# wwood/smafa

Hardware: AMD Instinct MI355X
Metric: query seqs/sec (DB residues/sec in `residues_per_s`) vs roofline, 10M x 60aa DB, d<=5 (higher is better)
Workload: dtype u32

## Files before the change

### smafa_amd/csrc/kernels.hip.h

```cpp
#pragma once

#include <type_traits>
#include <hip/hip_runtime.h>
#include <stdint.h>

#include "../../include/smafa_amd.h"
#include "scan_plan.h"

namespace smafa {

constexpr int kStageRows = 256;
__host__ __device__ constexpr int scan_min_waves(int ps, int w, int t) {
    const int regs = t * ps * w * 4 + 40;
    return regs <= 64 ? 8 : regs <= 80 ? 6 : regs <= 96 ? 5 : regs <= 128 ? 4 : regs <= 168 ? 3 : 2;
}
#ifndef SMAFA_CASCADE
#define SMAFA_CASCADE 1
#endif
#ifndef SMAFA_WIDE_AND_PAIR
#define SMAFA_WIDE_AND_PAIR 1
#endif
#ifndef SMAFA_SIGN_COMPARE
#define SMAFA_SIGN_COMPARE 1
#endif
// ... 863 lines not shown
#pragma unroll
        for (int t = 0; t < T; t++) {
            const bool live = (uint32_t)t < n_live;
            uint4 f1;
            if constexpr (kF1Home == 2) f1 = f1_reg[t];
            else f1 = planes[(size_t)(live ? tile0 + t : a.tile_begin) * (PS * W * 64) + (FP * W + 1) * 64 + lane];
            if constexpr (kF1Home == 1) f1_home[t * 64 + lane] = f1;
            const uint32_t w0[4] = {f0[t].x, f0[t].y, f0[t].z, f0[t].w};
            const uint32_t w1[4] = {f1.x, f1.y, f1.z, f1.w};
#pragma unroll
            for (int k = 0; k < 4; k++) {
                const uint32_t ky = key_y(w0[k]), kx = key_x(w1[k]);
                atomicOr(&km[(t * NS + 0) * KW + (ky >> 5)], 1u << (ky & 31u));
                atomicOr(&km[(t * NS + 1) * KW + (kx >> 5)], 1u << (kx & 31u));
                if (NS > 2) {
                    const uint32_t kz = key_z(w1[k]);
                    atomicOr(&km[(t * NS + (NS > 2 ? 2 : 0)) * KW + (kz >> 5)], 1u << (kz & 31u));
                }
            }
        }
        __builtin_amdgcn_wave_barrier();
        asm volatile("s_waitcnt lgkmcnt(0)" ::: "memory");
    }

    auto dma = [&](int b, uint32_t qc) {
        const uint32_t nqc = SMAFA_ZONE_FULL_DMA ? (uint32_t)kChunk : min((uint32_t)kChunk, q1 - qc);
        const uint4 *src = reinterpret_cast<const uint4 *>(qrec + (size_t)qc * RS);
#pragma unroll
        for (int v = 0; v < NV; v++) {
            const uint32_t idx = tid + v * NT;
            if (idx < nqc * RV)
                __builtin_amdgcn_global_load_lds((const __attribute__((address_space(1))) void *)(src + idx),
                                                 (__attribute__((address_space(3))) void *)(&stage[b][wave * 64 + v * NT]), 16, 0, 0);
        }
    };
    const uint32_t nu0 = ~a.thr0;
    auto load_bound = [&](uint32_t qc) -> uint32_t {
        return tid < min((uint32_t)kChunk, q1 - qc) ? ~ld_relaxed(a.thr + qc + tid) : 0u;
    };
    uint32_t nu_next = 0;
    auto read_record = [&](const uint4 *rec, uint32_t(&qw)[RS]) {
#pragma unroll
        for (int v = 0; v < RV; v++) {
            const uint4 x = rec[v];
            qw[4 * v + 0] = x.x;
            qw[4 * v + 1] = x.y;
            qw[4 * v + 2] = x.z;
            qw[4 * v + 3] = x.w;
        }
    };
    auto stream_compare = [&](uint32_t tile, const uint32_t(&qw)[RS], uint32_t q, int parity) {
        const uint32_t U = ~qw[BS];
        const uint4 *src = planes + (size_t)tile * (PS * W * 64) + lane;
        uint32_t d[4] = {0u, 0u, 0u, 0u};
#pragma unroll
        for (int w = 0; w < W; w++) {
            uint32_t extra = 0;
#pragma unroll
            for (int p = PS; p < PQ; p++) extra |= qw[qslot(PQ, W, p, w)];
            uint32_t m0 = extra, m1 = extra, m2 = extra, m3 = extra;
#pragma unroll
            for (int p = 0; p < PS; p++) {
                const uint4 v = src[(p * W + w) * 64];
                const uint32_t qv = qw[qslot(PQ, W, p, w)];
                m0 = or_xor(m0, v.x, qv);
                m1 = or_xor(m1, v.y, qv);
                m2 = or_xor(m2, v.z, qv);
                m3 = or_xor(m3, v.w, qv);
            }
            d[0] += __builtin_popcount(m0);
            d[1] += __builtin_popcount(m1);
            d[2] += __builtin_popcount(m2);
            d[3] += __builtin_popcount(m3);
        }
        const uint32_t subj0 = tile * kWaveTile + lane * 4u;
#pragma unroll
        for (int k = 0; k < 4; k++)
            if (d[k] <= U && subj0 + k < a.n_subjects) {
                if (DIRECT) emit_direct(a, q, subj0 + k, d[k]);
                else emit(a, rs, parity, q, subj0 + k, d[k]);
            }
    };
    auto load_head = [&](uint32_t qc) -> uint2 {
        return *reinterpret_cast<const uint2 *>(qrec + (size_t)(qc + lane) * RS);
    };
    uint2 head_next = make_uint2(0u, 0u);

    if (!DIRECT) {
        if (q0 < q1) {
            dma(0, q0);
            if (!FIXED && tid < (uint32_t)kChunk) nu_lds[0][tid] = load_bound(q0);
        }
        asm volatile("s_waitcnt vmcnt(0)" ::: "memory");
        __syncthreads();
    } else if (q0 < q1) {
        head_next = load_head(q0);
    }
    bool filter_on = a.use_filter != 0;
    uint32_t chunk_no = 0;
    for (uint32_t qc = q0; qc < q1; qc += kChunk, buf ^= 1, chunk_no++) {
        const uint32_t nqc = min((uint32_t)kChunk, q1 - qc);
        const bool more = qc + kChunk < q1;
        const uint2 head_cur = head_next;
        if (more) {
            if (DIRECT) {
                head_next = load_head(qc + kChunk);
            } else {
                dma(buf ^ 1, qc + kChunk);
                if (!FIXED) nu_next = load_bound(qc + kChunk);
            }
        }
        if (active) {
            const bool probe = a.use_filter && (filter_on || (chunk_no & 15u) == 0);
            if (probe) {
                uint32_t passes = 0;
                uint4 head = make_uint4(0u, 0u, 0u, 0u);
                if (DIRECT) head.x = head_cur.x, head.y = head_cur.y;
                else if (lane < nqc) head = stage[buf][lane * RV];
                const uint32_t hq0 = head.x, hq1 = W > 1 ? head.y : 0u;
                const uint32_t hnu = lane < nqc ? (FIXED ? nu0 : nu_lds[buf][lane]) : 0u;
                uint32_t nl = n_live;
                asm volatile("" : "+s"(nl));
                if (!SMAFA_ZONE_SGPR_ZONE) asm volatile("" : "+v"(vz.x), "+v"(vz.y));
                auto zone_keys = [&](auto slot) -> unsigned long long {
                    constexpr uint32_t t = decltype(slot)::value;
                    const uint32_t zc = SMAFA_ZONE_SGPR_ZONE ? zc0[t] : (uint32_t)__builtin_amdgcn_readlane((int)vz.x, (int)t);
                    const uint32_t zm = SMAFA_ZONE_SGPR_ZONE ? zm0[t] : (uint32_t)__builtin_amdgcn_readlane((int)vz.y, (int)t);
                    const uint32_t d0 = (hq0 ^ zc) & (kMaskInVgpr ? zmv[t] : zm);
                    uint32_t u = __builtin_popcount(d0) + hnu;
                    uint32_t d1 = 0;
                    if (zone_w1) {
                        const uint32_t zc1 = NS > 0 ? zc1s[t] : (uint32_t)__builtin_amdgcn_readlane((int)vz.z, (int)t);
                        const uint32_t zm1 = NS > 0 ? zm1s[t] : (uint32_t)__builtin_amdgcn_readlane((int)vz.w, (int)t);
                        d1 = (hq1 ^ zc1) & zm1;
                        u += __builtin_popcount(d1);
                    }
                    unsigned long long m = __ballot((int32_t)u < 0);
                    if constexpr (NS > 0) {
                        if ((uint32_t)__builtin_popcountll(m) >= a.key_gate) {
                            bool pass = false;
                            if ((int32_t)u < 0) {
                                const uint32_t s0 = hq0 ^ d0, s1 = hq1 ^ d1;
                                const uint32_t ky = key_y(s0), kx = key_x(s1);
                                const uint32_t vy = km[(t * NS + 0) * KW + (ky >> 5)];
                                const uint32_t vx = km[(t * NS + 1) * KW + (kx >> 5)];
                                uint32_t found = ((vy >> (ky & 31u)) & 1u) + ((vx >> (kx & 31u)) & 1u);
                                if (NS > 2) {
                                    const uint32_t kz = key_z(s1);
                                    const uint32_t vz_ = km[(t * NS + (NS > 2 ? 2 : 0)) * KW + (kz >> 5)];
                                    found += (vz_ >> (kz & 31u)) & 1u;
                                }
                                pass = found + ~u >= (uint32_t)NS;
                            }
                            m = __ballot(pass);
                        }
                    }
                    return m;
                };
                auto survivors = [&](auto slot, unsigned long long m) {
                    constexpr uint32_t t = decltype(slot)::value;
                    const uint32_t tile = tile0 + t;
                    const uint4 ft = f0[t];
                    while (m != 0ull) {
                        const int i = __builtin_ctzll(m);
                        asm("s_bitset0_b64 %0, %1" : "+s"(m) : "s"(i));
                        const uint32_t q0w = (uint32_t)__builtin_amdgcn_readlane((int)hq0, i);
                        const uint32_t nu = FIXED ? nu0 : (uint32_t)__builtin_amdgcn_readlane((int)hnu, i);
                        const uint32_t u0 = __builtin_popcount(ft.x ^ q0w) + nu;
                        const uint32_t u1 = __builtin_popcount(ft.y ^ q0w) + nu;
                        const uint32_t u2 = __builtin_popcount(ft.z ^ q0w) + nu;
                        const uint32_t u3 = __builtin_popcount(ft.w ^ q0w) + nu;
                        if (__ballot((int32_t)(or3(u0, u1, u2) | u3) < 0) == 0ull) continue;
                        uint32_t tile_r = tile;
                        asm volatile("" : "+s"(tile_r));
#if SMAFA_ZONE_OPAQUE_BUF
                        int buf_r = __builtin_amdgcn_readfirstlane(buf);
                        asm volatile("" : "+s"(buf_r));
#define SMAFA_ZONE_BUF buf_r
#else
#define SMAFA_ZONE_BUF buf
#endif
                        uint32_t qw[RS];
                        if constexpr (kL2Lanes) {
                            const uint32_t q1w = (uint32_t)__builtin_amdgcn_readlane((int)hq1, i);
                            uint4 v;
                            if constexpr (kF1Home == 1) v = f1_home[t * 64 + lane];
                            else if constexpr (kF1Home == 2) v = f1_reg[t];
                            else v = planes[(size_t)tile_r * (PS * W * 64) + (FP * W + 1) * 64 + lane];
                            const uint32_t m0 = or_xor(ft.x ^ q0w, v.x, q1w), m1 = or_xor(ft.y ^ q0w, v.y, q1w);
                            const uint32_t m2 = or_xor(ft.z ^ q0w, v.z, q1w), m3 = or_xor(ft.w ^ q0w, v.w, q1w);
                            if (kPair) {
                                const uint32_t sign = (__builtin_popcount(m0 & m1) + nu) | (__builtin_popcount(m2 & m3) + nu);
                                if (__ballot((int32_t)sign < 0) == 0ull) continue;
                            }
                            const uint32_t each = or3(__builtin_popcount(m0) + nu, __builtin_popcount(m1) + nu,
                                                      __builtin_popcount(m2) + nu) |
                                                  (__builtin_popcount(m3) + nu);
                            if (__ballot((int32_t)each < 0) == 0ull) continue;
                            read_record(reinterpret_cast<const uint4 *>(qrec + (size_t)(qc + (uint32_t)i) * RS), qw);
                            qw[BS] = nu;
                            passes++;
                            stream_compare(tile_r, qw, qc + (uint32_t)i, SMAFA_ZONE_BUF);
                            continue;
                        }
                        if (DIRECT) read_record(reinterpret_cast<const uint4 *>(qrec + (size_t)(qc + (uint32_t)i) * RS), qw);
                        else read_record(&stage[SMAFA_ZONE_BUF][(uint32_t)i * RV], qw);
                        qw[BS] = nu;
                        uint32_t m0 = ft.x ^ qw[0], m1 = ft.y ^ qw[0], m2 = ft.z ^ qw[0], m3 = ft.w ^ qw[0];
                        if (W > 1) {
                            const uint4 *src = planes + (size_t)tile_r * (PS * W * 64) + (FP * W) * 64 + lane;
#pragma unroll
                            for (int w = 1; w < W; w++) {
                                const uint4 v = src[w * 64];
                                m0 = or_xor(m0, v.x, qw[qslot(PQ, W, FP, w)]);
                                m1 = or_xor(m1, v.y, qw[qslot(PQ, W, FP, w)]);
                                m2 = or_xor(m2, v.z, qw[qslot(PQ, W, FP, w)]);
                                m3 = or_xor(m3, v.w, qw[qslot(PQ, W, FP, w)]);
                            }
                            if (kPair) {
                                const uint32_t sign = (__builtin_popcount(m0 & m1) + nu) | (__builtin_popcount(m2 & m3) + nu);
                                if (__ballot((int32_t)sign < 0) == 0ull) continue;
                            }
                            const uint32_t each = or3(__builtin_popcount(m0) + nu, __builtin_popcount(m1) + nu,
                                                      __builtin_popcount(m2) + nu) |
                                                  (__builtin_popcount(m3) + nu);
                            if (__ballot((int32_t)each < 0) == 0ull) continue;
                        }
                        passes++;
                        stream_compare(tile_r, qw, qc + (uint32_t)i, SMAFA_ZONE_BUF);
#undef SMAFA_ZONE_BUF
                    }
                };
                static_assert(T <= 8, "tile slots are spelled out below");
                auto each_slot = [&](auto &&f) {
                    f(std::integral_constant<uint32_t, 0>{});
                    if constexpr (T > 1) f(std::integral_constant<uint32_t, 1>{});
                    if constexpr (T > 2) f(std::integral_constant<uint32_t, 2>{});
                    if constexpr (T > 3) f(std::integral_constant<uint32_t, 3>{});
                    if constexpr (T > 4) f(std::integral_constant<uint32_t, 4>{});
                    if constexpr (T > 5) f(std::integral_constant<uint32_t, 5>{});
                    if constexpr (T > 6) f(std::integral_constant<uint32_t, 6>{});
                    if constexpr (T > 7) f(std::integral_constant<uint32_t, 7>{});
                };
                static_assert(!kHoist || (SMAFA_ZONE_NLIVE && SMAFA_ZONE_SGPR_ZONE),
                              "the two-phase form of the key-test kernels is written for SMAFA_ZONE_NLIVE = SMAFA_ZONE_SGPR_ZONE = 1");
                if constexpr (kHoist) {
                    unsigned long long ms[T];
                    if (key_hoist) {
                        const uint32_t ky = key_y(hq0), kx = key_x(hq1), kz = NS > 2 ? key_z(hq1) : 0u;
                        typedef const __attribute__((address_space(3))) uint32_t *lds_u32;
                        const uint32_t km_lds = (uint32_t)(uintptr_t)(__attribute__((address_space(3))) void *)km;
                        auto word_of = [&](uint32_t key) -> uint32_t {
                            uint32_t at;
                            asm("v_lshl_add_u32 %0, %1, 2, %2" : "=v"(at) : "v"(key >> 5), "s"(km_lds));
                            return at;
                        };
                        const uint32_t ay = word_of(ky), ax = word_of(kx), az = NS > 2 ? word_of(kz) : 0u;
                        const unsigned long long in_block = ~0ull >> (64u - nqc);
                        auto hoisted = [&](auto with_w1) {
                            if constexpr (SMAFA_ZONE_KEY_BATCH) {
                                uint32_t u[T];
                                bool test = false;
                                each_slot([&](auto slot) {
                                    constexpr uint32_t t = decltype(slot)::value;
                                    u[t] = __builtin_popcount((hq0 ^ zc0[t]) & (kMaskInVgpr ? zmv[t] : zm0[t])) + nu0;
                                    if (decltype(with_w1)::value) u[t] += __builtin_popcount((hq1 ^ zc1s[t]) & zm1s[t]);
                                    const unsigned long long m = __builtin_amdgcn_ballot_w64((int32_t)u[t] < 0) & in_block;
                                    ms[t] = t == 0u || nl > t ? m : 0ull;
                                    test = test || (uint32_t)__builtin_popcountll(ms[t]) >= a.key_gate;
                                });
                                if (test) {
                                    uint32_t g[T][3];
                                    each_slot([&](auto slot) {
                                        constexpr uint32_t t = decltype(slot)::value;
                                        g[t][0] = g[t][1] = g[t][2] = 0u;
                                        if ((int32_t)u[t] < 0) {
                                            g[t][0] = *(lds_u32)(uintptr_t)(ay + ((t * NS + 0) * KW) * 4u);
                                            g[t][1] = *(lds_u32)(uintptr_t)(ax + ((t * NS + 1) * KW) * 4u);
                                            if (NS > 2) g[t][2] = *(lds_u32)(uintptr_t)(az + ((t * NS + (NS > 2 ? 2 : 0)) * KW) * 4u);
                                        }
                                    });
                                    each_slot([&](auto slot) {
                                        constexpr uint32_t t = decltype(slot)::value;
                                        uint32_t found = __builtin_amdgcn_ubfe(g[t][0], ky, 1) + __builtin_amdgcn_ubfe(g[t][1], kx, 1);
                                        if (NS > 2) found += __builtin_amdgcn_ubfe(g[t][2], kz, 1);
                                        ms[t] &= __builtin_amdgcn_ballot_w64((int32_t)(u[t] - found) < -(int32_t)NS);
                                    });
                                }
                            } else {
                            auto one = [&](auto slot) -> unsigned long long {
                                constexpr uint32_t t = decltype(slot)::value;
                                uint32_t u = __builtin_popcount((hq0 ^ zc0[t]) & (kMaskInVgpr ? zmv[t] : zm0[t])) + nu0;
                                if (decltype(with_w1)::value) u += __builtin_popcount((hq1 ^ zc1s[t]) & zm1s[t]);
                                unsigned long long m = __builtin_amdgcn_ballot_w64((int32_t)u < 0) & in_block;
                                if ((uint32_t)__builtin_popcountll(m) >= a.key_gate) {
                                    if ((int32_t)u < 0) {
                                        uint32_t found = __builtin_amdgcn_ubfe(*(lds_u32)(uintptr_t)(ay + ((t * NS + 0) * KW) * 4u), ky, 1) +
                                                         __builtin_amdgcn_ubfe(*(lds_u32)(uintptr_t)(ax + ((t * NS + 1) * KW) * 4u), kx, 1);
                                        if (NS > 2) found += __builtin_amdgcn_ubfe(*(lds_u32)(uintptr_t)(az + ((t * NS + (NS > 2 ? 2 : 0)) * KW) * 4u), kz, 1);
                                        u -= found;
                                    }
                                    asm("" : "+v"(u));
                                    m &= __builtin_amdgcn_ballot_w64((int32_t)u < -(int32_t)NS);
                                }
                                return m;
                            };
                            each_slot([&](auto slot) {
                                constexpr uint32_t t = decltype(slot)::value;
                                ms[t] = t == 0u || nl > t ? one(slot) : 0ull;
                            });
                            }
                        };
                        if (zone_w1) hoisted(std::true_type{});
                        else hoisted(std::false_type{});
                    } else {
                        each_slot([&](auto slot) {
                            constexpr uint32_t t = decltype(slot)::value;
                            ms[t] = t == 0u || nl > t ? zone_keys(slot) : 0ull;
                        });
                    }
                    each_slot([&](auto slot) { survivors(slot, ms[decltype(slot)::value]); });
                } else {
                    each_slot([&](auto slot) {
                        constexpr uint32_t t = decltype(slot)::value;
                        if (SMAFA_ZONE_NLIVE ? nl > t : tile0 + t < a.tile_end) survivors(slot, zone_keys(slot));
                    });
                }
                filter_on = passes * 5u <= nqc * 8u;
            } else {
                for (uint32_t t = 0; t < (uint32_t)T; t++) {
                    const uint32_t tile = tile0 + t;
                    if (SMAFA_ZONE_NLIVE ? t >= n_live : tile >= a.tile_end) break;
                    uint4 s[PS * W];
                    uint32_t tile_d = tile;
                    asm volatile("" : "+s"(tile_d));
                    const uint4 *src = planes + (size_t)(SMAFA_ZONE_NLIVE ? tile_d : tile) * (PS * W * 64) + lane;
#pragma unroll
                    for (int i = 0; i < PS * W; i++) s[i] = src[i * 64];
                    const uint4 *rec = DIRECT ? reinterpret_cast<const uint4 *>(qrec + (size_t)qc * RS) : &stage[buf][0];
                    for (uint32_t i = 0; i < nqc; i++, rec += RV) {
                        uint32_t qw[RS];
                        read_record(rec, qw);
                        const uint32_t U = FIXED ? a.thr0 : ~nu_lds[buf][i];
                        uint32_t d[4];
#pragma unroll
                        for (int w = 0; w < W; w++) {
                            uint32_t extra = 0;
#pragma unroll
                            for (int p = PS; p < PQ; p++) extra |= qw[qslot(PQ, W, p, w)];
                            uint32_t m0 = extra, m1 = extra, m2 = extra, m3 = extra;
#pragma unroll
                            for (int p = 0; p < PS; p++) {
                                const uint4 v = s[p * W + w];
                                const uint32_t qv = qw[qslot(PQ, W, p, w)];
                                m0 = or_xor(m0, v.x, qv);
                                m1 = or_xor(m1, v.y, qv);
                                m2 = or_xor(m2, v.z, qv);
                                m3 = or_xor(m3, v.w, qv);
                            }
                            d[0] = (w ? d[0] : 0u) + __builtin_popcount(m0);
                            d[1] = (w ? d[1] : 0u) + __builtin_popcount(m1);
                            d[2] = (w ? d[2] : 0u) + __builtin_popcount(m2);
                            d[3] = (w ? d[3] : 0u) + __builtin_popcount(m3);
                        }
                        const uint32_t subj0 = tile * kWaveTile + lane * 4u;
#pragma unroll
                        for (int k = 0; k < 4; k++)
                            if (d[k] <= U && subj0 + k < a.n_subjects) {
                                if (DIRECT) emit_direct(a, qc + i, subj0 + k, d[k]);
                                else emit(a, rs, buf, qc + i, subj0 + k, d[k]);
                            }
                    }
                }
                load_filter();
            }
        }
        if (!DIRECT) {
            if (more && !FIXED && tid < (uint32_t)kChunk) nu_lds[buf ^ 1][tid] = nu_next;
            asm volatile("s_waitcnt vmcnt(0)" ::: "memory");
            __syncthreads();
            if (a.hits) flush_rows(a, rs, buf);
        }
    }
    finish_rows(a);
}

template <int PS, int PQ, int W>
__global__ __launch_bounds__(256) void scan_zone_few_kernel(const uint4 *__restrict__ planes,
                                                            const uint32_t *__restrict__ qrec, ScanArgs a) {
    constexpr int T = kFewTiles;
    constexpr int RS = qrec_stride(PQ, W);
    constexpr int RV = RS / 4;
    constexpr int FP = filter_plane(PQ);
    constexpr int BS = bound_slot(W);
    constexpr bool kPair = SMAFA_AND_PAIR && W > 1;
    __shared__ RowStage rs;
    const uint32_t tid = threadIdx.x;
    const uint32_t lane = tid & 63u;
    const uint32_t wave = tid >> 6;
    if (tid == 0) rs.n[0] = rs.n[1] = 0;
    __syncthreads();
    const uint32_t tile0 = (uint32_t)__builtin_amdgcn_readfirstlane((int)(a.tile_begin + (blockIdx.x * kWgWaves + wave) * T));
    const uint32_t nq = a.q_end - a.q_begin;
    if (tile0 < a.tile_end) {
        uint4 vz = make_uint4(0u, 0u, 0u, 0u);
        if (lane < (uint32_t)T && tile0 + lane < a.tile_end) vz = a.zone[tile0 + lane];
        uint4 head = make_uint4(0u, 0u, 0u, 0u);
        uint32_t hnu = 0;
        if (lane < nq) {
            head = reinterpret_cast<const uint4 *>(qrec + (size_t)(a.q_begin + lane) * RS)[0];
            hnu = ~(a.thr ? ld_relaxed(a.thr + a.q_begin + lane) : a.thr0);
        }
        const uint32_t hq0 = head.x, hq1 = W > 1 ? head.y : 0u;
        unsigned long long pass[T];
        uint4 f0[T];
#pragma unroll
        for (int t = 0; t < T; t++) {
            const uint32_t zc0 = (uint32_t)__builtin_amdgcn_readlane((int)vz.x, t);
            const uint32_t zm0 = (uint32_t)__builtin_amdgcn_readlane((int)vz.y, t);
            uint32_t u = __builtin_popcount((hq0 ^ zc0) & zm0) + hnu;
            if (W > 1) {
                const uint32_t zc1 = (uint32_t)__builtin_amdgcn_readlane((int)vz.z, t);
                const uint32_t zm1 = (uint32_t)__builtin_amdgcn_readlane((int)vz.w, t);
                u += __builtin_popcount((hq1 ^ zc1) & zm1);
            }
            pass[t] = tile0 + t < a.tile_end ? __ballot((int32_t)u < 0) : 0ull;
            if (pass[t] != 0ull) {
                f0[t] = planes[(size_t)(tile0 + t) * (PS * W * 64) + (FP * W) * 64 + lane];
            }
        }
#pragma unroll 1
        for (uint32_t t = 0; t < (uint32_t)T; t++) {
            unsigned long long m = 0ull;
            uint4 ft = f0[0];
#pragma unroll
            for (int k = 0; k < T; k++)
                if (t == (uint32_t)k) {
                    m = pass[k];
                    ft = f0[k];
                }
            const uint32_t tile = tile0 + t;
            while (m != 0ull) {
                const int i = __builtin_ctzll(m);
                m &= m - 1ull;
                const uint32_t q0w = (uint32_t)__builtin_amdgcn_readlane((int)hq0, i);
                const uint32_t nu = (uint32_t)__builtin_amdgcn_readlane((int)hnu, i);
                const uint32_t u0 = __builtin_popcount(ft.x ^ q0w) + nu;
                const uint32_t u1 = __builtin_popcount(ft.y ^ q0w) + nu;
                const uint32_t u2 = __builtin_popcount(ft.z ^ q0w) + nu;
                const uint32_t u3 = __builtin_popcount(ft.w ^ q0w) + nu;
                if (__ballot((int32_t)(or3(u0, u1, u2) | u3) < 0) == 0ull) continue;
                const uint32_t q = a.q_begin + (uint32_t)i;
                uint32_t qw[RS];
                const uint4 *rec = reinterpret_cast<const uint4 *>(qrec + (size_t)q * RS);
#pragma unroll
                for (int v = 0; v < RV; v++) {
                    const uint4 x = rec[v];
                    qw[4 * v + 0] = x.x;
                    qw[4 * v + 1] = x.y;
                    qw[4 * v + 2] = x.z;
                    qw[4 * v + 3] = x.w;
                }
                qw[BS] = nu;
                uint32_t m0 = ft.x ^ qw[0], m1 = ft.y ^ qw[0], m2 = ft.z ^ qw[0], m3 = ft.w ^ qw[0];
#pragma unroll
// ... 864 lines not shown
```

Before: 24.36 million.

## Split zone-scan chunk loop into full/plain specialised variants with batched key test

```diff
diff --git a/smafa_amd/csrc/kernels.hip.h b/smafa_amd/csrc/kernels.hip.h
--- a/smafa_amd/csrc/kernels.hip.h
+++ b/smafa_amd/csrc/kernels.hip.h
@@ -969,7 +969,9 @@
             }
     };
     auto load_head = [&](uint32_t qc) -> uint2 {
-        return *reinterpret_cast<const uint2 *>(qrec + (size_t)(qc + lane) * RS);
+        uint32_t l = lane;
+        if constexpr (kHoist) asm volatile("v_mbcnt_lo_u32_b32 %0, -1, 0\n\tv_mbcnt_hi_u32_b32 %0, -1, %0" : "=v"(l));
+        return *reinterpret_cast<const uint2 *>(qrec + (size_t)(qc + l) * RS);
     };
     uint2 head_next = make_uint2(0u, 0u);
 
@@ -985,289 +987,30 @@
     }
     bool filter_on = a.use_filter != 0;
     uint32_t chunk_no = 0;
-    for (uint32_t qc = q0; qc < q1; qc += kChunk, buf ^= 1, chunk_no++) {
-        const uint32_t nqc = min((uint32_t)kChunk, q1 - qc);
-        const bool more = qc + kChunk < q1;
-        const uint2 head_cur = head_next;
-        if (more) {
-            if (DIRECT) {
-                head_next = load_head(qc + kChunk);
-            } else {
-                dma(buf ^ 1, qc + kChunk);
-                if (!FIXED) nu_next = load_bound(qc + kChunk);
-            }
-        }
-        if (active) {
-            const bool probe = a.use_filter && (filter_on || (chunk_no & 15u) == 0);
-            if (probe) {
-                uint32_t passes = 0;
-                uint4 head = make_uint4(0u, 0u, 0u, 0u);
-                if (DIRECT) head.x = head_cur.x, head.y = head_cur.y;
-                else if (lane < nqc) head = stage[buf][lane * RV];
-                const uint32_t hq0 = head.x, hq1 = W > 1 ? head.y : 0u;
-                const uint32_t hnu = lane < nqc ? (FIXED ? nu0 : nu_lds[buf][lane]) : 0u;
-                uint32_t nl = n_live;
-                asm volatile("" : "+s"(nl));
-                if (!SMAFA_ZONE_SGPR_ZONE) asm volatile("" : "+v"(vz.x), "+v"(vz.y));
-                auto zone_keys = [&](auto slot) -> unsigned long long {
-                    constexpr uint32_t t = decltype(slot)::value;
-                    const uint32_t zc = SMAFA_ZONE_SGPR_ZONE ? zc0[t] : (uint32_t)__builtin_amdgcn_readlane((int)vz.x, (int)t);
-                    const uint32_t zm = SMAFA_ZONE_SGPR_ZONE ? zm0[t] : (uint32_t)__builtin_amdgcn_readlane((int)vz.y, (int)t);
-                    const uint32_t d0 = (hq0 ^ zc) & (kMaskInVgpr ? zmv[t] : zm);
-                    uint32_t u = __builtin_popcount(d0) + hnu;
-                    uint32_t d1 = 0;
-                    if (zone_w1) {
-                        const uint32_t zc1 = NS > 0 ? zc1s[t] : (uint32_t)__builtin_amdgcn_readlane((int)vz.z, (int)t);
-                        const uint32_t zm1 = NS > 0 ? zm1s[t] : (uint32_t)__builtin_amdgcn_readlane((int)vz.w, (int)t);
-                        d1 = (hq1 ^ zc1) & zm1;
-                        u += __builtin_popcount(d1);
-                    }
-                    unsigned long long m = __ballot((int32_t)u < 0);
-                    if constexpr (NS > 0) {
-                        if ((uint32_t)__builtin_popcountll(m) >= a.key_gate) {
-                            bool pass = false;
-                            if ((int32_t)u < 0) {
-                                const uint32_t s0 = hq0 ^ d0, s1 = hq1 ^ d1;
-                                const uint32_t ky = key_y(s0), kx = key_x(s1);
-                                const uint32_t vy = km[(t * NS + 0) * KW + (ky >> 5)];
-                                const uint32_t vx = km[(t * NS + 1) * KW + (kx >> 5)];
-                                uint32_t found = ((vy >> (ky & 31u)) & 1u) + ((vx >> (kx & 31u)) & 1u);
-                                if (NS > 2) {
-                                    const uint32_t kz = key_z(s1);
-                                    const uint32_t vz_ = km[(t * NS + (NS > 2 ? 2 : 0)) * KW + (kz >> 5)];
-                                    found += (vz_ >> (kz & 31u)) & 1u;
-                                }
-                                pass = found + ~u >= (uint32_t)NS;
-                            }
-                            m = __ballot(pass);
-                        }
-                    }
-                    return m;
-                };
-                auto survivors = [&](auto slot, unsigned long long m) {
-                    constexpr uint32_t t = decltype(slot)::value;
-                    const uint32_t tile = tile0 + t;
-                    const uint4 ft = f0[t];
-                    while (m != 0ull) {
-                        const int i = __builtin_ctzll(m);
-                        asm("s_bitset0_b64 %0, %1" : "+s"(m) : "s"(i));
-                        const uint32_t q0w = (uint32_t)__builtin_amdgcn_readlane((int)hq0, i);
-                        const uint32_t nu = FIXED ? nu0 : (uint32_t)__builtin_amdgcn_readlane((int)hnu, i);
-                        const uint32_t u0 = __builtin_popcount(ft.x ^ q0w) + nu;
-                        const uint32_t u1 = __builtin_popcount(ft.y ^ q0w) + nu;
-                        const uint32_t u2 = __builtin_popcount(ft.z ^ q0w) + nu;
-                        const uint32_t u3 = __builtin_popcount(ft.w ^ q0w) + nu;
-                        if (__ballot((int32_t)(or3(u0, u1, u2) | u3) < 0) == 0ull) continue;
-                        uint32_t tile_r = tile;
-                        asm volatile("" : "+s"(tile_r));
-#if SMAFA_ZONE_OPAQUE_BUF
-                        int buf_r = __builtin_amdgcn_readfirstlane(buf);
-                        asm volatile("" : "+s"(buf_r));
-#define SMAFA_ZONE_BUF buf_r
-#else
-#define SMAFA_ZONE_BUF buf
-#endif
-                        uint32_t qw[RS];
-                        if constexpr (kL2Lanes) {
-                            const uint32_t q1w = (uint32_t)__builtin_amdgcn_readlane((int)hq1, i);
-                            uint4 v;
-                            if constexpr (kF1Home == 1) v = f1_home[t * 64 + lane];
-                            else if constexpr (kF1Home == 2) v = f1_reg[t];
-                            else v = planes[(size_t)tile_r * (PS * W * 64) + (FP * W + 1) * 64 + lane];
-                            const uint32_t m0 = or_xor(ft.x ^ q0w, v.x, q1w), m1 = or_xor(ft.y ^ q0w, v.y, q1w);
-                            const uint32_t m2 = or_xor(ft.z ^ q0w, v.z, q1w), m3 = or_xor(ft.w ^ q0w, v.w, q1w);
-                            if (kPair) {
-                                const uint32_t sign = (__builtin_popcount(m0 & m1) + nu) | (__builtin_popcount(m2 & m3) + nu);
-                                if (__ballot((int32_t)sign < 0) == 0ull) continue;
-                            }
-                            const uint32_t each = or3(__builtin_popcount(m0) + nu, __builtin_popcount(m1) + nu,
-                                                      __builtin_popcount(m2) + nu) |
-                                                  (__builtin_popcount(m3) + nu);
-                            if (__ballot((int32_t)each < 0) == 0ull) continue;
-                            read_record(reinterpret_cast<const uint4 *>(qrec + (size_t)(qc + (uint32_t)i) * RS), qw);
-                            qw[BS] = nu;
-                            passes++;
-                            stream_compare(tile_r, qw, qc + (uint32_t)i, SMAFA_ZONE_BUF);
-                            continue;
-                        }
-                        if (DIRECT) read_record(reinterpret_cast<const uint4 *>(qrec + (size_t)(qc + (uint32_t)i) * RS), qw);
-                        else read_record(&stage[SMAFA_ZONE_BUF][(uint32_t)i * RV], qw);
-                        qw[BS] = nu;
-                        uint32_t m0 = ft.x ^ qw[0], m1 = ft.y ^ qw[0], m2 = ft.z ^ qw[0], m3 = ft.w ^ qw[0];
-                        if (W > 1) {
-                            const uint4 *src = planes + (size_t)tile_r * (PS * W * 64) + (FP * W) * 64 + lane;
-#pragma unroll
-                            for (int w = 1; w < W; w++) {
-                                const uint4 v = src[w * 64];
-                                m0 = or_xor(m0, v.x, qw[qslot(PQ, W, FP, w)]);
-                                m1 = or_xor(m1, v.y, qw[qslot(PQ, W, FP, w)]);
-                                m2 = or_xor(m2, v.z, qw[qslot(PQ, W, FP, w)]);
-                                m3 = or_xor(m3, v.w, qw[qslot(PQ, W, FP, w)]);
-                            }
-                            if (kPair) {
-                                const uint32_t sign = (__builtin_popcount(m0 & m1) + nu) | (__builtin_popcount(m2 & m3) + nu);
-                                if (__ballot((int32_t)sign < 0) == 0ull) continue;
-                            }
-                            const uint32_t each = or3(__builtin_popcount(m0) + nu, __builtin_popcount(m1) + nu,
-                                                      __builtin_popcount(m2) + nu) |
-                                                  (__builtin_popcount(m3) + nu);
-                            if (__ballot((int32_t)each < 0) == 0ull) continue;
-                        }
-                        passes++;
-                        stream_compare(tile_r, qw, qc + (uint32_t)i, SMAFA_ZONE_BUF);
-#undef SMAFA_ZONE_BUF
-                    }
-                };
-                static_assert(T <= 8, "tile slots are spelled out below");
-                auto each_slot = [&](auto &&f) {
-                    f(std::integral_constant<uint32_t, 0>{});
-                    if constexpr (T > 1) f(std::integral_constant<uint32_t, 1>{});
-                    if constexpr (T > 2) f(std::integral_constant<uint32_t, 2>{});
-                    if constexpr (T > 3) f(std::integral_constant<uint32_t, 3>{});
-                    if constexpr (T > 4) f(std::integral_constant<uint32_t, 4>{});
-                    if constexpr (T > 5) f(std::integral_constant<uint32_t, 5>{});
-                    if constexpr (T > 6) f(std::integral_constant<uint32_t, 6>{});
-                    if constexpr (T > 7) f(std::integral_constant<uint32_t, 7>{});
-                };
-                static_assert(!kHoist || (SMAFA_ZONE_NLIVE && SMAFA_ZONE_SGPR_ZONE),
-                              "the two-phase form of the key-test kernels is written for SMAFA_ZONE_NLIVE = SMAFA_ZONE_SGPR_ZONE = 1");
-                if constexpr (kHoist) {
-                    unsigned long long ms[T];
-                    if (key_hoist) {
-                        const uint32_t ky = key_y(hq0), kx = key_x(hq1), kz = NS > 2 ? key_z(hq1) : 0u;
-                        typedef const __attribute__((address_space(3))) uint32_t *lds_u32;
-                        const uint32_t km_lds = (uint32_t)(uintptr_t)(__attribute__((address_space(3))) void *)km;
-                        auto word_of = [&](uint32_t key) -> uint32_t {
-                            uint32_t at;
-                            asm("v_lshl_add_u32 %0, %1, 2, %2" : "=v"(at) : "v"(key >> 5), "s"(km_lds));
-                            return at;
-                        };
-                        const uint32_t ay = word_of(ky), ax = word_of(kx), az = NS > 2 ? word_of(kz) : 0u;
-                        const unsigned long long in_block = ~0ull >> (64u - nqc);
-                        auto hoisted = [&](auto with_w1) {
-                            if constexpr (SMAFA_ZONE_KEY_BATCH) {
-                                uint32_t u[T];
-                                bool test = false;
-                                each_slot([&](auto slot) {
-                                    constexpr uint32_t t = decltype(slot)::value;
-                                    u[t] = __builtin_popcount((hq0 ^ zc0[t]) & (kMaskInVgpr ? zmv[t] : zm0[t])) + nu0;
-                                    if (decltype(with_w1)::value) u[t] += __builtin_popcount((hq1 ^ zc1s[t]) & zm1s[t]);
-                                    const unsigned long long m = __builtin_amdgcn_ballot_w64((int32_t)u[t] < 0) & in_block;
-                                    ms[t] = t == 0u || nl > t ? m : 0ull;
-                                    test = test || (uint32_t)__builtin_popcountll(ms[t]) >= a.key_gate;
-                                });
-                                if (test) {
-                                    uint32_t g[T][3];
-                                    each_slot([&](auto slot) {
-                                        constexpr uint32_t t = decltype(slot)::value;
-                                        g[t][0] = g[t][1] = g[t][2] = 0u;
-                                        if ((int32_t)u[t] < 0) {
-                                            g[t][0] = *(lds_u32)(uintptr_t)(ay + ((t * NS + 0) * KW) * 4u);
-                                            g[t][1] = *(lds_u32)(uintptr_t)(ax + ((t * NS + 1) * KW) * 4u);
-                                            if (NS > 2) g[t][2] = *(lds_u32)(uintptr_t)(az + ((t * NS + (NS > 2 ? 2 : 0)) * KW) * 4u);
-                                        }
-                                    });
-                                    each_slot([&](auto slot) {
-                                        constexpr uint32_t t = decltype(slot)::value;
-                                        uint32_t found = __builtin_amdgcn_ubfe(g[t][0], ky, 1) + __builtin_amdgcn_ubfe(g[t][1], kx, 1);
-                                        if (NS > 2) found += __builtin_amdgcn_ubfe(g[t][2], kz, 1);
-                                        ms[t] &= __builtin_amdgcn_ballot_w64((int32_t)(u[t] - found) < -(int32_t)NS);
-                                    });
-                                }
-                            } else {
-                            auto one = [&](auto slot) -> unsigned long long {
-                                constexpr uint32_t t = decltype(slot)::value;
-                                uint32_t u = __builtin_popcount((hq0 ^ zc0[t]) & (kMaskInVgpr ? zmv[t] : zm0[t])) + nu0;
-                                if (decltype(with_w1)::value) u += __builtin_popcount((hq1 ^ zc1s[t]) & zm1s[t]);
-                                unsigned long long m = __builtin_amdgcn_ballot_w64((int32_t)u < 0) & in_block;
-                                if ((uint32_t)__builtin_popcountll(m) >= a.key_gate) {
-                                    if ((int32_t)u < 0) {
-                                        uint32_t found = __builtin_amdgcn_ubfe(*(lds_u32)(uintptr_t)(ay + ((t * NS + 0) * KW) * 4u), ky, 1) +
-                                                         __builtin_amdgcn_ubfe(*(lds_u32)(uintptr_t)(ax + ((t * NS + 1) * KW) * 4u), kx, 1);
-                                        if (NS > 2) found += __builtin_amdgcn_ubfe(*(lds_u32)(uintptr_t)(az + ((t * NS + (NS > 2 ? 2 : 0)) * KW) * 4u), kz, 1);
-                                        u -= found;
-                                    }
-                                    asm("" : "+v"(u));
-                                    m &= __builtin_amdgcn_ballot_w64((int32_t)u < -(int32_t)NS);
-                                }
-                                return m;
-                            };
-                            each_slot([&](auto slot) {
-                                constexpr uint32_t t = decltype(slot)::value;
-                                ms[t] = t == 0u || nl > t ? one(slot) : 0ull;
-                            });
-                            }
-                        };
-                        if (zone_w1) hoisted(std::true_type{});
-                        else hoisted(std::false_type{});
-                    } else {
-                        each_slot([&](auto slot) {
-                            constexpr uint32_t t = decltype(slot)::value;
-                            ms[t] = t == 0u || nl > t ? zone_keys(slot) : 0ull;
-                        });
-                    }
-                    each_slot([&](auto slot) { survivors(slot, ms[decltype(slot)::value]); });
-                } else {
-                    each_slot([&](auto slot) {
-                        constexpr uint32_t t = decltype(slot)::value;
-                        if (SMAFA_ZONE_NLIVE ? nl > t : tile0 + t < a.tile_end) survivors(slot, zone_keys(slot));
-                    });
-                }
-                filter_on = passes * 5u <= nqc * 8u;
-            } else {
-                for (uint32_t t = 0; t < (uint32_t)T; t++) {
-                    const uint32_t tile = tile0 + t;
-                    if (SMAFA_ZONE_NLIVE ? t >= n_live : tile >= a.tile_end) break;
-                    uint4 s[PS * W];
-                    uint32_t tile_d = tile;
-                    asm volatile("" : "+s"(tile_d));
-                    const uint4 *src = planes + (size_t)(SMAFA_ZONE_NLIVE ? tile_d : tile) * (PS * W * 64) + lane;
-#pragma unroll
-                    for (int i = 0; i < PS * W; i++) s[i] = src[i * 64];
-                    const uint4 *rec = DIRECT ? reinterpret_cast<const uint4 *>(qrec + (size_t)qc * RS) : &stage[buf][0];
-                    for (uint32_t i = 0; i < nqc; i++, rec += RV) {
-                        uint32_t qw[RS];
-                        read_record(rec, qw);
-                        const uint32_t U = FIXED ? a.thr0 : ~nu_lds[buf][i];
-                        uint32_t d[4];
-#pragma unroll
-                        for (int w = 0; w < W; w++) {
-                            uint32_t extra = 0;
-#pragma unroll
-                            for (int p = PS; p < PQ; p++) extra |= qw[qslot(PQ, W, p, w)];
-                            uint32_t m0 = extra, m1 = extra, m2 = extra, m3 = extra;
-#pragma unroll
-                            for (int p = 0; p < PS; p++) {
-                                const uint4 v = s[p * W + w];
-                                const uint32_t qv = qw[qslot(PQ, W, p, w)];
-                                m0 = or_xor(m0, v.x, qv);
-                                m1 = or_xor(m1, v.y, qv);
-                                m2 = or_xor(m2, v.z, qv);
-                                m3 = or_xor(m3, v.w, qv);
-                            }
-                            d[0] = (w ? d[0] : 0u) + __builtin_popcount(m0);
-                            d[1] = (w ? d[1] : 0u) + __builtin_popcount(m1);
-                            d[2] = (w ? d[2] : 0u) + __builtin_popcount(m2);
-                            d[3] = (w ? d[3] : 0u) + __builtin_popcount(m3);
-                        }
-                        const uint32_t subj0 = tile * kWaveTile + lane * 4u;
-#pragma unroll
-                        for (int k = 0; k < 4; k++)
-                            if (d[k] <= U && subj0 + k < a.n_subjects) {
-                                if (DIRECT) emit_direct(a, qc + i, subj0 + k, d[k]);
-                                else emit(a, rs, buf, qc + i, subj0 + k, d[k]);
-                            }
-                    }
-                }
-                load_filter();
-            }
-        }
-        if (!DIRECT) {
-            if (more && !FIXED && tid < (uint32_t)kChunk) nu_lds[buf ^ 1][tid] = nu_next;
-            asm volatile("s_waitcnt vmcnt(0)" ::: "memory");
-            __syncthreads();
-            if (a.hits) flush_rows(a, rs, buf);
-        }
+    constexpr bool kSplit = kHoist;
+    const uint32_t qb0 = kSplit ? (uint32_t)__builtin_amdgcn_readfirstlane((int)q0) : q0;
+    const uint32_t qb1 = kSplit ? (uint32_t)__builtin_amdgcn_readfirstlane((int)q1) : q1;
+    if constexpr (!kSplit) {
+        for (uint32_t qc = q0; qc < q1; qc += kChunk, buf ^= 1, chunk_no++) {
+            constexpr bool PLAIN = false, FULL = false;
+#include "zone_chunk.inc.h"
+        }
+    } else if (active && qb0 < qb1) {
+        uint32_t qc = qb0;
+        auto chunk_pass = [&](auto plain_c, auto full_c) {
+            constexpr bool PLAIN = decltype(plain_c)::value, FULL = decltype(full_c)::value;
+#include "zone_chunk.inc.h"
+        };
+        constexpr std::true_type yes{};
+        constexpr std::false_type no{};
+        const bool plain_wave = a.use_filter != 0 && key_hoist && !zone_w1 && n_live == (uint32_t)T;
+        if (plain_wave) {
+            while (filter_on && qc + kChunk < qb1) {
+                chunk_pass(yes, yes);
+                qc += kChunk;
+            }
+        }
+        for (; qc < qb1; qc += kChunk) chunk_pass(no, no);
     }
     finish_rows(a);
 }
diff --git a/smafa_amd/csrc/zone_chunk.inc.h b/smafa_amd/csrc/zone_chunk.inc.h
--- /dev/null
+++ b/smafa_amd/csrc/zone_chunk.inc.h
@@ -0,0 +1,301 @@
+        const uint32_t nqc = FULL ? (uint32_t)kChunk : min((uint32_t)kChunk, qb1 - qc);
+        const bool more = FULL || qc + kChunk < qb1;
+        const uint2 head_cur = head_next;
+        if (more) {
+            if (DIRECT) {
+                head_next = load_head(qc + kChunk);
+            } else {
+                dma(buf ^ 1, qc + kChunk);
+                if (!FIXED) nu_next = load_bound(qc + kChunk);
+            }
+        }
+        if (PLAIN || active) {
+            const uint32_t cn = kSplit ? (qc - qb0) / (uint32_t)kChunk : chunk_no;
+            const bool probe = PLAIN || (a.use_filter && (filter_on || (cn & 15u) == 0));
+            if (probe) {
+                uint32_t passes = 0;
+                uint4 head = make_uint4(0u, 0u, 0u, 0u);
+                if (DIRECT) head.x = head_cur.x, head.y = head_cur.y;
+                else if (lane < nqc) head = stage[buf][lane * RV];
+                const uint32_t hq0 = head.x, hq1 = W > 1 ? head.y : 0u;
+                const uint32_t hnu = lane < nqc ? (FIXED ? nu0 : nu_lds[buf][lane]) : 0u;
+                uint32_t nl = PLAIN ? (uint32_t)T : n_live;
+                if constexpr (!PLAIN) asm volatile("" : "+s"(nl));
+                if (!SMAFA_ZONE_SGPR_ZONE) asm volatile("" : "+v"(vz.x), "+v"(vz.y));
+                auto zone_keys = [&](auto slot) -> unsigned long long {
+                    constexpr uint32_t t = decltype(slot)::value;
+                    const uint32_t zc = SMAFA_ZONE_SGPR_ZONE ? zc0[t] : (uint32_t)__builtin_amdgcn_readlane((int)vz.x, (int)t);
+                    const uint32_t zm = SMAFA_ZONE_SGPR_ZONE ? zm0[t] : (uint32_t)__builtin_amdgcn_readlane((int)vz.y, (int)t);
+                    const uint32_t d0 = (hq0 ^ zc) & (kMaskInVgpr ? zmv[t] : zm);
+                    uint32_t u = __builtin_popcount(d0) + hnu;
+                    uint32_t d1 = 0;
+                    if (zone_w1) {
+                        const uint32_t zc1 = NS > 0 ? zc1s[t] : (uint32_t)__builtin_amdgcn_readlane((int)vz.z, (int)t);
+                        const uint32_t zm1 = NS > 0 ? zm1s[t] : (uint32_t)__builtin_amdgcn_readlane((int)vz.w, (int)t);
+                        d1 = (hq1 ^ zc1) & zm1;
+                        u += __builtin_popcount(d1);
+                    }
+                    unsigned long long m = __ballot((int32_t)u < 0);
+                    if constexpr (NS > 0) {
+                        if ((uint32_t)__builtin_popcountll(m) >= a.key_gate) {
+                            bool pass = false;
+                            if ((int32_t)u < 0) {
+                                const uint32_t s0 = hq0 ^ d0, s1 = hq1 ^ d1;
+                                const uint32_t ky = key_y(s0), kx = key_x(s1);
+                                const uint32_t vy = km[(t * NS + 0) * KW + (ky >> 5)];
+                                const uint32_t vx = km[(t * NS + 1) * KW + (kx >> 5)];
+                                uint32_t found = ((vy >> (ky & 31u)) & 1u) + ((vx >> (kx & 31u)) & 1u);
+                                if (NS > 2) {
+                                    const uint32_t kz = key_z(s1);
+                                    const uint32_t vz_ = km[(t * NS + (NS > 2 ? 2 : 0)) * KW + (kz >> 5)];
+                                    found += (vz_ >> (kz & 31u)) & 1u;
+                                }
+                                pass = found + ~u >= (uint32_t)NS;
+                            }
+                            m = __ballot(pass);
+                        }
+                    }
+                    return m;
+                };
+                auto survivors = [&](auto slot, unsigned long long m) {
+                    constexpr uint32_t t = decltype(slot)::value;
+                    const uint32_t tile = tile0 + t;
+                    const uint4 ft = f0[t];
+                    if constexpr (kSplit) {
+                        m = (unsigned long long)(uint32_t)__builtin_amdgcn_readfirstlane((int)(uint32_t)m) |
+                            (unsigned long long)(uint32_t)__builtin_amdgcn_readfirstlane((int)(uint32_t)(m >> 32)) << 32;
+                    }
+                    while (m != 0ull) {
+                        const int i = __builtin_ctzll(m);
+                        asm("s_bitset0_b64 %0, %1" : "+s"(m) : "s"(i));
+                        const uint32_t q0w = (uint32_t)__builtin_amdgcn_readlane((int)hq0, i);
+                        const uint32_t nu = FIXED ? nu0 : (uint32_t)__builtin_amdgcn_readlane((int)hnu, i);
+                        const uint32_t u0 = __builtin_popcount(ft.x ^ q0w) + nu;
+                        const uint32_t u1 = __builtin_popcount(ft.y ^ q0w) + nu;
+                        const uint32_t u2 = __builtin_popcount(ft.z ^ q0w) + nu;
+                        const uint32_t u3 = __builtin_popcount(ft.w ^ q0w) + nu;
+                        if (__ballot((int32_t)(or3(u0, u1, u2) | u3) < 0) == 0ull) continue;
+                        uint32_t tile_r = tile;
+                        asm volatile("" : "+s"(tile_r));
+#if SMAFA_ZONE_OPAQUE_BUF
+                        int buf_r = __builtin_amdgcn_readfirstlane(buf);
+                        asm volatile("" : "+s"(buf_r));
+#define SMAFA_ZONE_BUF buf_r
+#else
+#define SMAFA_ZONE_BUF buf
+#endif
+                        uint32_t qw[RS];
+                        if constexpr (kL2Lanes) {
+                            const uint32_t q1w = (uint32_t)__builtin_amdgcn_readlane((int)hq1, i);
+                            uint4 v;
+                            if constexpr (kF1Home == 1) v = f1_home[t * 64 + lane];
+                            else if constexpr (kF1Home == 2) v = f1_reg[t];
+                            else v = planes[(size_t)tile_r * (PS * W * 64) + (FP * W + 1) * 64 + lane];
+                            const uint32_t m0 = or_xor(ft.x ^ q0w, v.x, q1w), m1 = or_xor(ft.y ^ q0w, v.y, q1w);
+                            const uint32_t m2 = or_xor(ft.z ^ q0w, v.z, q1w), m3 = or_xor(ft.w ^ q0w, v.w, q1w);
+                            if (kPair) {
+                                const uint32_t sign = (__builtin_popcount(m0 & m1) + nu) | (__builtin_popcount(m2 & m3) + nu);
+                                if (__ballot((int32_t)sign < 0) == 0ull) continue;
+                            }
+                            const uint32_t each = or3(__builtin_popcount(m0) + nu, __builtin_popcount(m1) + nu,
+                                                      __builtin_popcount(m2) + nu) |
+                                                  (__builtin_popcount(m3) + nu);
+                            if (__ballot((int32_t)each < 0) == 0ull) continue;
+                            read_record(reinterpret_cast<const uint4 *>(qrec + (size_t)(qc + (uint32_t)i) * RS), qw);
+                            qw[BS] = nu;
+                            passes++;
+                            stream_compare(tile_r, qw, qc + (uint32_t)i, SMAFA_ZONE_BUF);
+                            continue;
+                        }
+                        if (DIRECT) read_record(reinterpret_cast<const uint4 *>(qrec + (size_t)(qc + (uint32_t)i) * RS), qw);
+                        else read_record(&stage[SMAFA_ZONE_BUF][(uint32_t)i * RV], qw);
+                        qw[BS] = nu;
+                        uint32_t m0 = ft.x ^ qw[0], m1 = ft.y ^ qw[0], m2 = ft.z ^ qw[0], m3 = ft.w ^ qw[0];
+                        if (W > 1) {
+                            const uint4 *src = planes + (size_t)tile_r * (PS * W * 64) + (FP * W) * 64 + lane;
+#pragma unroll
+                            for (int w = 1; w < W; w++) {
+                                const uint4 v = src[w * 64];
+                                m0 = or_xor(m0, v.x, qw[qslot(PQ, W, FP, w)]);
+                                m1 = or_xor(m1, v.y, qw[qslot(PQ, W, FP, w)]);
+                                m2 = or_xor(m2, v.z, qw[qslot(PQ, W, FP, w)]);
+                                m3 = or_xor(m3, v.w, qw[qslot(PQ, W, FP, w)]);
+                            }
+                            if (kPair) {
+                                const uint32_t sign = (__builtin_popcount(m0 & m1) + nu) | (__builtin_popcount(m2 & m3) + nu);
+                                if (__ballot((int32_t)sign < 0) == 0ull) continue;
+                            }
+                            const uint32_t each = or3(__builtin_popcount(m0) + nu, __builtin_popcount(m1) + nu,
+                                                      __builtin_popcount(m2) + nu) |
+                                                  (__builtin_popcount(m3) + nu);
+                            if (__ballot((int32_t)each < 0) == 0ull) continue;
+                        }
+                        passes++;
+                        stream_compare(tile_r, qw, qc + (uint32_t)i, SMAFA_ZONE_BUF);
+#undef SMAFA_ZONE_BUF
+                    }
+                };
+                static_assert(T <= 8, "tile slots are spelled out below");
+                auto each_slot = [&](auto &&f) {
+                    f(std::integral_constant<uint32_t, 0>{});
+                    if constexpr (T > 1) f(std::integral_constant<uint32_t, 1>{});
+                    if constexpr (T > 2) f(std::integral_constant<uint32_t, 2>{});
+                    if constexpr (T > 3) f(std::integral_constant<uint32_t, 3>{});
+                    if constexpr (T > 4) f(std::integral_constant<uint32_t, 4>{});
+                    if constexpr (T > 5) f(std::integral_constant<uint32_t, 5>{});
+                    if constexpr (T > 6) f(std::integral_constant<uint32_t, 6>{});
+                    if constexpr (T > 7) f(std::integral_constant<uint32_t, 7>{});
+                };
+                static_assert(!kHoist || (SMAFA_ZONE_NLIVE && SMAFA_ZONE_SGPR_ZONE),
+                              "the two-phase form of the key-test kernels is written for SMAFA_ZONE_NLIVE = SMAFA_ZONE_SGPR_ZONE = 1");
+                if constexpr (kHoist) {
+                    unsigned long long ms[T];
+                    if (PLAIN || key_hoist) {
+                        const uint32_t ky = key_y(hq0), kx = key_x(hq1), kz = NS > 2 ? key_z(hq1) : 0u;
+                        typedef const __attribute__((address_space(3))) uint32_t *lds_u32;
+                        const uint32_t km_lds = (uint32_t)(uintptr_t)(__attribute__((address_space(3))) void *)km;
+                        auto word_of = [&](uint32_t key) -> uint32_t {
+                            uint32_t at;
+                            asm("v_lshl_add_u32 %0, %1, 2, %2" : "=v"(at) : "v"(key >> 5), "s"(km_lds));
+                            return at;
+                        };
+                        const uint32_t ay = word_of(ky), ax = word_of(kx), az = NS > 2 ? word_of(kz) : 0u;
+                        const unsigned long long in_block = FULL ? ~0ull : ~0ull >> (64u - nqc);
+                        auto hoisted = [&](auto with_w1) {
+                            if constexpr (SMAFA_ZONE_KEY_BATCH) {
+                                uint32_t u[T];
+                                bool test = false;
+                                unsigned long long any = 0ull;
+                                each_slot([&](auto slot) {
+                                    constexpr uint32_t t = decltype(slot)::value;
+                                    u[t] = __builtin_popcount((hq0 ^ zc0[t]) & (kMaskInVgpr ? zmv[t] : zm0[t])) + nu0;
+                                    if (decltype(with_w1)::value) u[t] += __builtin_popcount((hq1 ^ zc1s[t]) & zm1s[t]);
+                                    unsigned long long m = __builtin_amdgcn_ballot_w64((int32_t)u[t] < 0);
+                                    if constexpr (!FULL) m &= in_block;
+                                    ms[t] = PLAIN || t == 0u || nl > t ? m : 0ull;
+                                    if constexpr (PLAIN) any |= m;
+                                    else test = test || (uint32_t)__builtin_popcountll(ms[t]) >= a.key_gate;
+                                });
+                                if constexpr (PLAIN) test = (uint32_t)__builtin_popcountll(any) >= a.key_gate;
+                                if (test) {
+                                    uint32_t g[T][3];
+                                    each_slot([&](auto slot) {
+                                        constexpr uint32_t t = decltype(slot)::value;
+                                        if constexpr (PLAIN) asm volatile("" : "=v"(g[t][0]), "=v"(g[t][1]), "=v"(g[t][2]));
+                                        else g[t][0] = g[t][1] = g[t][2] = 0u;
+                                        if ((int32_t)u[t] < 0) {
+                                            g[t][0] = *(lds_u32)(uintptr_t)(ay + ((t * NS + 0) * KW) * 4u);
+                                            g[t][1] = *(lds_u32)(uintptr_t)(ax + ((t * NS + 1) * KW) * 4u);
+                                            if (NS > 2) g[t][2] = *(lds_u32)(uintptr_t)(az + ((t * NS + (NS > 2 ? 2 : 0)) * KW) * 4u);
+                                        }
+                                    });
+                                    each_slot([&](auto slot) {
+                                        constexpr uint32_t t = decltype(slot)::value;
+                                        uint32_t found = __builtin_amdgcn_ubfe(g[t][0], ky, 1) + __builtin_amdgcn_ubfe(g[t][1], kx, 1);
+                                        if (NS > 2) found += __builtin_amdgcn_ubfe(g[t][2], kz, 1);
+                                        ms[t] &= __builtin_amdgcn_ballot_w64((int32_t)(u[t] - found) < -(int32_t)NS);
+                                    });
+                                }
+                            } else {
+                            auto one = [&](auto slot) -> unsigned long long {
+                                constexpr uint32_t t = decltype(slot)::value;
+                                uint32_t u = __builtin_popcount((hq0 ^ zc0[t]) & (kMaskInVgpr ? zmv[t] : zm0[t])) + nu0;
+                                if (decltype(with_w1)::value) u += __builtin_popcount((hq1 ^ zc1s[t]) & zm1s[t]);
+                                unsigned long long m = __builtin_amdgcn_ballot_w64((int32_t)u < 0) & in_block;
+                                if ((uint32_t)__builtin_popcountll(m) >= a.key_gate) {
+                                    if ((int32_t)u < 0) {
+                                        uint32_t found = __builtin_amdgcn_ubfe(*(lds_u32)(uintptr_t)(ay + ((t * NS + 0) * KW) * 4u), ky, 1) +
+                                                         __builtin_amdgcn_ubfe(*(lds_u32)(uintptr_t)(ax + ((t * NS + 1) * KW) * 4u), kx, 1);
+                                        if (NS > 2) found += __builtin_amdgcn_ubfe(*(lds_u32)(uintptr_t)(az + ((t * NS + (NS > 2 ? 2 : 0)) * KW) * 4u), kz, 1);
+                                        u -= found;
+                                    }
+                                    asm("" : "+v"(u));
+                                    m &= __builtin_amdgcn_ballot_w64((int32_t)u < -(int32_t)NS);
+                                }
+                                return m;
+                            };
+                            each_slot([&](auto slot) {
+                                constexpr uint32_t t = decltype(slot)::value;
+                                ms[t] = t == 0u || nl > t ? one(slot) : 0ull;
+                            });
+                            }
+                        };
+                        if (!PLAIN && zone_w1) hoisted(std::true_type{});
+                        else hoisted(std::false_type{});
+                    } else {
+                        each_slot([&](auto slot) {
+                            constexpr uint32_t t = decltype(slot)::value;
+                            ms[t] = t == 0u || nl > t ? zone_keys(slot) : 0ull;
+                        });
+                    }
+                    each_slot([&](auto slot) { survivors(slot, ms[decltype(slot)::value]); });
+                } else {
+                    each_slot([&](auto slot) {
+                        constexpr uint32_t t = decltype(slot)::value;
+                        if (SMAFA_ZONE_NLIVE ? nl > t : tile0 + t < a.tile_end) survivors(slot, zone_keys(slot));
+                    });
+                }
+                if constexpr (kSplit) {
+                    const uint32_t n_exact = (uint32_t)__builtin_amdgcn_readfirstlane((int)passes);
+                    if constexpr (PLAIN) {
+                        if (n_exact * 5u > nqc * 8u) filter_on = false;
+                    } else {
+                        filter_on = n_exact * 5u <= nqc * 8u;
+                    }
+                } else {
+                    filter_on = passes * 5u <= nqc * 8u;
+                }
+            } else {
+                for (uint32_t t = 0; t < (uint32_t)T; t++) {
+                    const uint32_t tile = tile0 + t;
+                    if (SMAFA_ZONE_NLIVE ? t >= n_live : tile >= a.tile_end) break;
+                    uint4 s[PS * W];
+                    uint32_t tile_d = tile;
+                    asm volatile("" : "+s"(tile_d));
+                    const uint4 *src = planes + (size_t)(SMAFA_ZONE_NLIVE ? tile_d : tile) * (PS * W * 64) + lane;
+#pragma unroll
+                    for (int i = 0; i < PS * W; i++) s[i] = src[i * 64];
+                    const uint4 *rec = DIRECT ? reinterpret_cast<const uint4 *>(qrec + (size_t)qc * RS) : &stage[buf][0];
+                    for (uint32_t i = 0; i < nqc; i++, rec += RV) {
+                        uint32_t qw[RS];
+                        read_record(rec, qw);
+                        const uint32_t U = FIXED ? a.thr0 : ~nu_lds[buf][i];
+                        uint32_t d[4];
+#pragma unroll
+                        for (int w = 0; w < W; w++) {
+                            uint32_t extra = 0;
+#pragma unroll
+                            for (int p = PS; p < PQ; p++) extra |= qw[qslot(PQ, W, p, w)];
+                            uint32_t m0 = extra, m1 = extra, m2 = extra, m3 = extra;
+#pragma unroll
+                            for (int p = 0; p < PS; p++) {
+                                const uint4 v = s[p * W + w];
+                                const uint32_t qv = qw[qslot(PQ, W, p, w)];
+                                m0 = or_xor(m0, v.x, qv);
+                                m1 = or_xor(m1, v.y, qv);
+                                m2 = or_xor(m2, v.z, qv);
+                                m3 = or_xor(m3, v.w, qv);
+                            }
+                            d[0] = (w ? d[0] : 0u) + __builtin_popcount(m0);
+                            d[1] = (w ? d[1] : 0u) + __builtin_popcount(m1);
+                            d[2] = (w ? d[2] : 0u) + __builtin_popcount(m2);
+                            d[3] = (w ? d[3] : 0u) + __builtin_popcount(m3);
+                        }
+                        const uint32_t subj0 = tile * kWaveTile + lane * 4u;
+#pragma unroll
+                        for (int k = 0; k < 4; k++)
+                            if (d[k] <= U && subj0 + k < a.n_subjects) {
+                                if (DIRECT) emit_direct(a, qc + i, subj0 + k, d[k]);
+                                else emit(a, rs, buf, qc + i, subj0 + k, d[k]);
+                            }
+                    }
+                }
+                load_filter();
+            }
+        }
+        if (!DIRECT) {
+            if (more && !FIXED && tid < (uint32_t)kChunk) nu_lds[buf ^ 1][tid] = nu_next;
+            asm volatile("s_waitcnt vmcnt(0)" ::: "memory");
+            __syncthreads();
+            if (a.hits) flush_rows(a, rs, buf);
+        }
```

After: 29.90 million (median of 6 runs). +22.8%, better.
